# A2R-Lab/RBDReference

Hardware: AMD Instinct MI355X
Metric: batched RNEA+grad evals/s (7-DoF) (higher is better)
Workload: dtype f32

## Files before the change

rbdreference_amd/csrc/rbd_idsva_pipe.h:

```cpp
#pragma once
#include "rbd_idsva.h"

namespace rbdk {

constexpr bool ids_pipe_ok_() {
  if (!GRAD_IDSVA_OK) return false;
  if (n_groups() != 1 || grad_max_rows() != N) return false;
  if (N < 4) return false;
  if ((32 * GRAD_TILE) % 4 != 0 || GRAD_TILE % 2 != 0) return false;
  return true;
}
constexpr bool IDS_PIPE_OK = ids_pipe_ok_();

#define IDS_SB() __builtin_amdgcn_sched_barrier(0)
#ifndef IDS_FDG_LOAD_AT
#define IDS_FDG_LOAD_AT 0
#endif
#ifndef IDS_PIPE_LEAF_PARK
#define IDS_PIPE_LEAF_PARK 0
#endif
#ifndef IDS_PIPE_C_PARK
#define IDS_PIPE_C_PARK 0
#endif
#ifndef IDS_PIPE_PARK_UPTO
#define IDS_PIPE_PARK_UPTO 0
#endif
#ifndef IDS_PIPE_REG_ENTRIES_MAX
#define IDS_PIPE_REG_ENTRIES_MAX 50
#endif
constexpr int ids_pipe_rows_a(int rows) {
  for (int a = 0; a < rows; ++a)
    if (ids_regs_for(rows, a) <= IDS_PIPE_REG_ENTRIES_MAX && ids_tile_for(rows, a) <= IDS_TS) return a;
  return ids_rows_a(rows);
}
template <class X>
RBD_DEV void ids_undef(X& x) { asm volatile("" : "=v"(x)); }

template <class T, bool HAS_QDD, bool FDG = false>
__global__ __launch_bounds__(64, 2) void rnea_grad_idsva_pipe_kernel(const T* __restrict__ q, const T* __restrict__ qd,
                                                                    const T* __restrict__ qdd, T grav, int use_damping,
                                                                    long long B, T* __restrict__ c_out,
                                                                    T* __restrict__ dcdu, const T* __restrict__ minv_pk) {
  static_assert(sizeof(T) == 4, "fp32 kernel");
  extern __shared__ __attribute__((aligned(16))) unsigned char smem_raw[];
  T* tile = reinterpret_cast<T*>(smem_raw);
  const int lane = threadIdx.x;
  constexpr int CFGS = 64;
  constexpr int TS = IDS_TS;
  constexpr int row0 = 0, rows = N, last = N - 1;
  constexpr int ra = ids_pipe_rows_a(rows);
  static_assert(ids_tile_for(rows, ra) <= IDS_TS, "tile overflow");
  constexpr int rs = rows - ra;
  constexpr int PEND = ra * GRAD_ROW;
  constexpr int RW = GRAD_TILE;
  constexpr int VE = 4;
  constexpr int NV = 32 * RW / VE;
  constexpr int NRD = (NV + 63) / 64;
  constexpr int NVC = CFGS * N / VE;
  constexpr int NRC = (NVC + 63) / 64;
  typedef T V __attribute__((ext_vector_type(VE)));
  const long long ntiles = (B + CFGS - 1) / CFGS;
  long long t = blockIdx.x;
  if (t >= ntiles) return;
  T* my = tile + lane * TS;
  int gdim = (int)gridDim.x;
  asm volatile("" : "+s"(gdim));

  JTrig<T> tr[N];
  T qv[N], qdv[N], qddv[N];
  T qn[N], qdn[N], qddn[N];
  T Sv[N][6], Pd[N][6], Pdd[N][6];
  T cv[N];
  T Rm[3][3], pw[3], v[6], a[6];
  T E[RW];
  T mk[FDG ? FDC_NP : 1];
  long long tcur = 0;

  auto load_inputs = [&](long long tt, bool dummy) {
    const long long c0 = tt * CFGS;
    const long long rm = dummy ? 1 : B - c0;
    unsigned lo = (unsigned)((lane < rm ? lane : (int)rm - 1) * N);
    asm volatile("" : "+v"(lo));
    const T* qt = q + c0 * N + lo;
    const T* qdt = qd + c0 * N + lo;
    const T* qddt = HAS_QDD ? qdd + c0 * N + lo : nullptr;
    sfor<0, N>([&](auto J) {
      constexpr int j = decltype(J)::value;
      qn[j] = qt[j];
      qdn[j] = qdt[j];
      if constexpr (HAS_QDD) qddn[j] = qddt[j]; else qddn[j] = T(0);
    });
  };
  auto settle_inputs = [&]() {
    sfor<0, N>([&](auto J) {
      constexpr int j = decltype(J)::value;
      qn[j] = launder(qn[j]); qdn[j] = launder(qdn[j]); qddn[j] = launder(qddn[j]);
    });
  };
  auto take_inputs = [&]() {
    sfor<0, N>([&](auto J) { constexpr int j = decltype(J)::value; qv[j] = qn[j]; qdv[j] = qdn[j]; qddv[j] = qddn[j]; });
  };
  auto trig_chunk = [&](auto J0_, auto J1_) {
    constexpr int J0 = decltype(J0_)::value, J1 = decltype(J1_)::value;
    T mx = T(0);
    sfor<J0, J1>([&](auto J) { constexpr int j = decltype(J)::value; mx = __builtin_fmaxf(mx, __builtin_fabsf(qv[j])); });
    if (__builtin_expect(__builtin_amdgcn_ballot_w64(!(mx <= 8192.0f)) != 0, 0)) {
      sfor<J0, J1>([&](auto J) { constexpr int j = decltype(J)::value; sincos_wide_(qv[j], &tr[j].s, &tr[j].c); });
    } else {
      sfor<J0, J1>([&](auto J) { constexpr int j = decltype(J)::value; sincos_core_(qv[j], &tr[j].s, &tr[j].c); });
    }
  };

  auto fwd_body = [&](auto J) {
    constexpr int j = decltype(J)::value;
    constexpr int k = AXIS[j], ka = (k + 1) % 3, kb = (k + 2) % 3;
    constexpr bool root = PARENT[j] < 0;
    T Tm[3][3];
    sfor<0, 3>([&](auto R_) {
      sfor<0, 3>([&](auto C_) {
        constexpr int r = decltype(R_)::value, c = decltype(C_)::value;
        if constexpr (root) {
          Tm[r][c] = T(Et_(j, c, r));
        } else {
          T acc = T(0);
          sfor<0, 3>([&](auto M_) {
            constexpr int m = decltype(M_)::value;
            constexpr double e = Et_(j, c, m);
            if constexpr (e == 1.0) acc = acc + Rm[r][m];
            else if constexpr (e == -1.0) acc = acc - Rm[r][m];
            else if constexpr (e != 0.0) acc = fma_(T(e), Rm[r][m], acc);
          });
          Tm[r][c] = acc;
        }
      });
    });
    T pn[3];
    sfor<0, 3>([&](auto R_) {
      constexpr int r = decltype(R_)::value;
      if constexpr (root) {
        pn[r] = T(rt_(j, r));
      } else {
        T acc = pw[r];
        sfor<0, 3>([&](auto M_) {
          constexpr int m = decltype(M_)::value;
          constexpr double e = rt_(j, m);
          if constexpr (e != 0.0) acc = fma_(T(e), Rm[r][m], acc);
        });
        pn[r] = acc;
      }
    });
    sfor<0, 3>([&](auto R_) {
      constexpr int r = decltype(R_)::value;
      Rm[r][ka] = fma_(tr[j].c, Tm[r][ka], tr[j].s * Tm[r][kb]);
      Rm[r][kb] = fma_(tr[j].c, Tm[r][kb], -(tr[j].s * Tm[r][ka]));
      Rm[r][k] = Tm[r][k];
      pw[r] = pn[r];
    });
    const T ang[3] = {Rm[0][k], Rm[1][k], Rm[2][k]};
    T sl[3];
    cross3(pw, ang, sl);
    sfor<0, 3>([&](auto R_) { constexpr int r = decltype(R_)::value; Sv[j][r] = ang[r]; Sv[j][3 + r] = sl[r]; });
    if constexpr (root) {
      sfor<0, 6>([&](auto R_) { Pd[j][decltype(R_)::value] = T(0); });
      Pdd[j][0] = T(0); Pdd[j][1] = T(0); Pdd[j][2] = T(0);
      Pdd[j][3] = grav * ang[1];
      Pdd[j][4] = -(grav * ang[0]);
      Pdd[j][5] = T(0);
      sfor<0, 6>([&](auto R_) {
        constexpr int r = decltype(R_)::value;
        v[r] = Sv[j][r] * qdv[j];
        a[r] = Sv[j][r] * qddv[j];
      });
      a[5] -= grav;
    } else {
      T t1[6];
      crm6(v, Sv[j], Pd[j]);
      crm6(a, Sv[j], t1);
      crm6_add(v, Pd[j], t1, Pdd[j]);
      sfor<0, 6>([&](auto R_) {
        constexpr int r = decltype(R_)::value;
        v[r] = fma_(Sv[j][r], qdv[j], v[r]);
        a[r] = fma_(Sv[j][r], qddv[j], fma_(Pd[j][r], qdv[j], a[r]));
      });
    }
  };
  auto park = [&](auto J) {
    constexpr int j = decltype(J)::value;
    if constexpr (j > row0 && j < last && j <= IDS_PIPE_PARK_UPTO) {
      my[ids_park_slot(row0, rows, ra, j, 0)] = tr[j].s; my[ids_park_slot(row0, rows, ra, j, 1)] = tr[j].c;
      my[ids_park_slot(row0, rows, ra, j, 2)] = qdv[j]; my[ids_park_slot(row0, rows, ra, j, 3)] = qddv[j];
    }
    if constexpr (j == last && (IDS_PIPE_LEAF_PARK && ids_leaf_parks(row0, rows, ra))) {
      my[ids_leaf_slot(row0, rows, ra, 0)] = tr[j].s; my[ids_leaf_slot(row0, rows, ra, 1)] = tr[j].c;
      my[ids_leaf_slot(row0, rows, ra, 2)] = qdv[j]; my[ids_leaf_slot(row0, rows, ra, 3)] = qddv[j];
    }
  };

  auto backward = [&](long long tnext_or_t, bool dummy) {
    RInertia<T> IC;
    SymB<T> SC;
    T pmC[6], fC[6];
    sfor_down<row0, row0 + rows>([&](auto J) {
      constexpr int j = decltype(J)::value;
      constexpr int k = AXIS[j], ka = (k + 1) % 3, kb = (k + 2) % 3;
      constexpr bool top = j >= rs;
      if constexpr (j == rs && ra > 1 && (IDS_PIPE_C_PARK && ids_c_parks(row0, rows, ra))) {
        asm volatile("" ::: "memory");
        sfor<rs + 1, row0 + rows>([&](auto JC) { constexpr int jc = decltype(JC)::value; cv[jc] = my[ids_c_slot(row0, rows, ra, jc - rs - 1)]; });
      }
      if constexpr (j > row0 && j < last && j <= IDS_PIPE_PARK_UPTO) {
        asm volatile("" ::: "memory");
        tr[j].s = my[ids_park_slot(row0, rows, ra, j, 0)]; tr[j].c = my[ids_park_slot(row0, rows, ra, j, 1)];
        qdv[j] = my[ids_park_slot(row0, rows, ra, j, 2)]; qddv[j] = my[ids_park_slot(row0, rows, ra, j, 3)];
#ifndef RBD_EXP_NO_PIN_READBACK
        IDS_SB();
#endif
      }
      if constexpr (FDG && j == row0 + (rows > IDS_FDG_LOAD_AT ? IDS_FDG_LOAD_AT : rows - 1)) {
        IDS_SB();
        int lo = lane;
        asm volatile("" : "+v"(lo));
        const T* mp = minv_pk + (size_t)tcur * (FDC_NP * 64) + lo;
#ifdef RBD_FDG_EXP_NOLOAD
        sfor<0, FDC_NP>([&](auto S_) { constexpr int s_ = decltype(S_)::value; mk[s_] = launder(T(1) + T(s_)); });
#else
        sfor<0, FDC_NP>([&](auto S_) { constexpr int s_ = decltype(S_)::value; mk[s_] = mp[s_ * 64]; });
#endif
        IDS_SB();
      }
      RInertia<T> L;
      T cw[3];
      sfor<0, 3>([&](auto R_) {
        constexpr int r = decltype(R_)::value;
        T acc = pw[r];
        sfor<0, 3>([&](auto M_) {
          constexpr int m = decltype(M_)::value;
          constexpr double e = com_(j, m);
          if constexpr (e != 0.0) acc = fma_(T(e), Rm[r][m], acc);
        });
        cw[r] = acc;
      });
      L.m = T(mass_(j));
      sfor<0, 3>([&](auto R_) { L.h[decltype(R_)::value] = T(mass_(j)) * cw[decltype(R_)::value]; });
      {
        T A[3][3];
        sfor<0, 3>([&](auto R_) {
          sfor<0, 3>([&](auto C_) {
            constexpr int r = decltype(R_)::value, c = decltype(C_)::value;
            T acc = T(0);
            sfor<0, 3>([&](auto M_) {
              constexpr int m = decltype(M_)::value;
              constexpr double e = Ic_(j, m, c);
              if constexpr (e != 0.0) acc = fma_(T(e), Rm[r][m], acc);
            });
            A[r][c] = acc;
          });
        });
        const T cc = fma_(cw[0], cw[0], fma_(cw[1], cw[1], cw[2] * cw[2]));
        constexpr int IR[6] = {0, 0, 0, 1, 1, 2}, IC_[6] = {0, 1, 2, 1, 2, 2};
        sfor<0, 6>([&](auto E_) {
          constexpr int e = decltype(E_)::value, r = IR[e], c = IC_[e];
          T s = fma_(A[r][0], Rm[c][0], fma_(A[r][1], Rm[c][1], A[r][2] * Rm[c][2]));
          s = fma_(-L.h[r], cw[c], s);
          if constexpr (r == c) s = fma_(L.m, cc, s);
          L.I[e] = s;
        });
      }
      T pm[6];
      rin_apply(L, v, pm);
      if constexpr (j == last) {
        T Ia[6];
        rin_apply(L, a, Ia);
        fxv_add(v, pm, Ia, fC);
        IC = L;
        sfor<0, 6>([&](auto R_) { constexpr int r = decltype(R_)::value; pmC[r] = pm[r]; });
      } else {
        T t[6];
        rin_apply_acc(L, a, fC, t);
        fxv_add(v, pm, t, fC);
        IC.m += L.m;
        sfor<0, 3>([&](auto R_) { constexpr int r = decltype(R_)::value; IC.h[r] += L.h[r]; });
        sfor<0, 6>([&](auto R_) { constexpr int r = decltype(R_)::value; IC.I[r] += L.I[r]; pmC[r] += pm[r]; });
      }
      {
        const T w[3] = {v[0], v[1], v[2]}, u[3] = {v[3], v[4], v[5]};
        const T Ifull[3][3] = {{L.I[0], L.I[1], L.I[2]}, {L.I[1], L.I[3], L.I[4]}, {L.I[2], L.I[4], L.I[5]}};
        const T uh = fma_(u[0], L.h[0], fma_(u[1], L.h[1], u[2] * L.h[2]));
        constexpr int IR[6] = {0, 0, 0, 1, 1, 2}, IC_[6] = {0, 1, 2, 1, 2, 2};
        sfor<0, 6>([&](auto E_) {
          constexpr int e = decltype(E_)::value, r = IR[e], c = IC_[e];
          constexpr int r1 = (r + 1) % 3, r2 = (r + 2) % 3, c1 = (c + 1) % 3, c2 = (c + 2) % 3;
          const T base = (j == last) ? T(0) : SC.TL[e];
          if constexpr (r == c) {
            const T d = fma_(-L.h[r], u[r], fma_(w[r1], Ifull[r2][r], fma_(-w[r2], Ifull[r1][r], uh)));
            SC.TL[e] = fma_(T(2), d, base);
          } else {
            T x = fma_(w[r1], Ifull[r2][c], fma_(-w[r2], Ifull[r1][c], base));
            x = fma_(w[c1], Ifull[c2][r], fma_(-w[c2], Ifull[c1][r], x));
            SC.TL[e] = fma_(-L.h[r], u[c], fma_(-u[r], L.h[c], x));
          }
        });
        sfor<0, 3>([&](auto R_) {
          constexpr int r = decltype(R_)::value, r1 = (r + 1) % 3, r2 = (r + 2) % 3;
          const T base = (j == last) ? T(0) : SC.G[r];
          SC.G[r] = fma_(L.m, u[r], fma_(w[r1], L.h[r2], fma_(-w[r2], L.h[r1], base)));
        });
      }
      cv[j] = dot6(Sv[j], fC);
      if constexpr (j > rs && (IDS_PIPE_C_PARK && ids_c_parks(row0, rows, ra))) my[ids_c_slot(row0, rows, ra, j - rs - 1)] = cv[j];
      T t1[6], t2[6], t3[6], t4[6];
      {
        T y3[6], s1[6], yf[6];
        rin_apply(IC, Sv[j], t1);
        sym_apply(SC, Sv[j], s1);
        fxv_sub(Sv[j], pmC, s1, t4);
        rin_apply(IC, Pdd[j], y3);
        fxv_add(Sv[j], fC, y3, yf);
        if constexpr (PARENT[j] < 0) {
          sfor<0, 6>([&](auto R_) {
            constexpr int r = decltype(R_)::value;
            t3[r] = yf[r];
            t2[r] = fma_(T(2), s1[r], -t4[r]);
          });
        } else {
          T y2[6], ys[6];
          rin_apply(IC, Pd[j], y2);
          sym_apply_acc(SC, Pd[j], yf, ys);
          fxv_add(Pd[j], pmC, ys, t3);
          sfor<0, 6>([&](auto R_) {
            constexpr int r = decltype(R_)::value;
            t2[r] = fma_(T(2), y2[r] + s1[r], -t4[r]);
          });
        }
      }
      sfor<row0, j + 1>([&](auto JJ) {
        constexpr int jj = decltype(JJ)::value;
        T dq_ij, dqd_ij;
        if constexpr (PARENT[jj] < 0) {
          dq_ij = fma_(t1[3], Pdd[jj][3], t1[4] * Pdd[jj][4]);
          dqd_ij = dot6(t4, Sv[jj]);
        } else {
          dq_ij = dot6_acc(t1, Pdd[jj], dot6(t4, Pd[jj]));
          dqd_ij = fma_(T(2), dot6(t1, Pd[jj]), dot6(t4, Sv[jj]));
        }
        if constexpr (jj == j) dqd_ij += sel(use_damping != 0, T(DAMPING[j]), T(0));
        if constexpr (top) {
          my[(j - rs) * GRAD_ROW + jj] = dq_ij;
          my[(j - rs) * GRAD_ROW + N + jj] = dqd_ij;
        } else {
          E[(j - row0) * GRAD_ROW + jj] = dq_ij;
          E[(j - row0) * GRAD_ROW + N + jj] = dqd_ij;
        }
        if constexpr (jj != j) {
          const T e3 = dot6(Sv[jj], t3), e2 = dot6(Sv[jj], t2);
          if constexpr (!top) {
            E[(jj - row0) * GRAD_ROW + j] = e3;
            E[(jj - row0) * GRAD_ROW + N + j] = e2;
          } else if constexpr (jj < rs) {
            constexpr int slot = PEND + ((jj - row0) * ra + (j - rs)) * 2;
            my[slot] = e3;
            my[slot + 1] = e2;
          } else {
            my[(jj - rs) * GRAD_ROW + j] = e3;
            my[(jj - rs) * GRAD_ROW + N + j] = e2;
          }
        }
      });
      if constexpr (j == row0 + (rows > IDS_PREFETCH_AT ? IDS_PREFETCH_AT : rows - 1)) {
        IDS_SB();
        load_inputs(tnext_or_t, dummy);
        IDS_SB();
      }
      if constexpr (j == last && (IDS_PIPE_LEAF_PARK && ids_leaf_parks(row0, rows, ra))) {
        asm volatile("" ::: "memory");
        tr[j].s = my[ids_leaf_slot(row0, rows, ra, 0)]; tr[j].c = my[ids_leaf_slot(row0, rows, ra, 1)];
        qdv[j] = my[ids_leaf_slot(row0, rows, ra, 2)]; qddv[j] = my[ids_leaf_slot(row0, rows, ra, 3)];
      }
      if constexpr (j > row0) {
        sfor<0, 6>([&](auto R_) {
          constexpr int r = decltype(R_)::value;
          v[r] = fma_(-Sv[j][r], qdv[j], v[r]);
          a[r] = fma_(-Sv[j][r], qddv[j], fma_(-Pd[j][r], qdv[j], a[r]));
        });
        T Tm[3][3];
        sfor<0, 3>([&](auto R_) {
          constexpr int r = decltype(R_)::value;
          Tm[r][ka] = fma_(tr[j].c, Rm[r][ka], -(tr[j].s * Rm[r][kb]));
          Tm[r][kb] = fma_(tr[j].s, Rm[r][ka], tr[j].c * Rm[r][kb]);
          Tm[r][k] = Rm[r][k];
        });
        sfor<0, 3>([&](auto R_) {
          sfor<0, 3>([&](auto C_) {
            constexpr int r = decltype(R_)::value, c = decltype(C_)::value;
            T acc = T(0);
            sfor<0, 3>([&](auto M_) {
              constexpr int m = decltype(M_)::value;
              constexpr double e = Et_(j, m, c);
              if constexpr (e == 1.0) acc = acc + Tm[r][m];
              else if constexpr (e == -1.0) acc = acc - Tm[r][m];
              else if constexpr (e != 0.0) acc = fma_(T(e), Tm[r][m], acc);
            });
            Rm[r][c] = acc;
          });
        });
        sfor<0, 3>([&](auto R_) {
          constexpr int r = decltype(R_)::value;
          T acc = pw[r];
          sfor<0, 3>([&](auto M_) {
            constexpr int m = decltype(M_)::value;
            constexpr double e = rt_(j, m);
            if constexpr (e != 0.0) acc = fma_(T(-e), Rm[r][m], acc);
          });
          pw[r] = acc;
        });
      }
    });
  };

  auto readback = [&]() {
    sfor<rs, row0 + rows>([&](auto R_) {
      sfor<0, GRAD_ROW>([&](auto C_) {
        constexpr int r = decltype(R_)::value, c = decltype(C_)::value;
        E[(r - row0) * GRAD_ROW + c] = my[(r - rs) * GRAD_ROW + c];
      });
    });
    sfor<row0, rs>([&](auto JJ) {
      sfor<rs, row0 + rows>([&](auto JA) {
        constexpr int jj = decltype(JJ)::value, ja = decltype(JA)::value;
        constexpr int slot = PEND + ((jj - row0) * ra + (ja - rs)) * 2;
        E[(jj - row0) * GRAD_ROW + ja] = my[slot];
        E[(jj - row0) * GRAD_ROW + N + ja] = my[slot + 1];
      });
    });
  };
  auto image_write = [&](int ln, int h) {
    if ((ln >> 5) == h) {
      T* img = tile + (ln & 31) * RW;
      typedef T V2 __attribute__((ext_vector_type(2)));
      sfor<0, RW / 2>([&](auto K_) {
        constexpr int k = decltype(K_)::value;
        V2 x; x[0] = E[2 * k]; x[1] = E[2 * k + 1];
        reinterpret_cast<V2*>(img)[k] = x;
      });
    }
  };
  auto image_read = [&](int ln, V (&buf)[NRD]) {
    const V* src = reinterpret_cast<const V*>(tile);
    sfor<0, NRD>([&](auto I_) {
      constexpr int i = decltype(I_)::value;
      if constexpr ((i + 1) * 64 <= NV) buf[i] = src[ln + 64 * i];
      else buf[i] = src[(ln + 64 * i < NV) ? ln + 64 * i : 0];
    });
  };
  auto image_store = [&](int ln, long long cfg0, int h, const V (&buf)[NRD]) {
    V* dst = reinterpret_cast<V*>(dcdu + (cfg0 + 32 * h) * GRAD_TILE);
    sfor<0, NRD>([&](auto I_) {
      constexpr int i = decltype(I_)::value;
      if constexpr ((i + 1) * 64 <= NV) dst[ln + 64 * i] = buf[i];
      else { if (ln + 64 * i < NV) dst[ln + 64 * i] = buf[i]; }
    });
  };
  auto flush_half_plain = [&](int ln, long long cfg0, int nvalid, int h) {
    image_write(ln, h);
    IDS_WAVE_SYNC();
    const int nv = nvalid - 32 * h;
    if (nv >= 32) {
      V buf[NRD];
      image_read(ln, buf);
      image_store(ln, cfg0, h, buf);
    } else if (nv > 0) {
      T* gdst = dcdu + (cfg0 + 32 * h) * GRAD_TILE;
#pragma unroll 2
      for (int g = ln; g < nv * RW; g += 64) gdst[g] = tile[g];
    }
    IDS_WAVE_SYNC();
  };
  auto flush_c_plain = [&](int ln, long long cfg0, int nvalid) {
    if (c_out != nullptr) {
      sfor<0, N>([&](auto J) { constexpr int j = decltype(J)::value; tile[ln * N + j] = cv[j]; });
      IDS_WAVE_SYNC();
      T* cdst = c_out + cfg0 * N;
      if (nvalid == CFGS && (CFGS * N) % VE == 0) {
        sfor<0, NRC>([&](auto I_) {
          constexpr int i = decltype(I_)::value;
          if (ln + 64 * i < NVC) reinterpret_cast<V*>(cdst)[ln + 64 * i] = reinterpret_cast<const V*>(tile)[ln + 64 * i];
        });
      } else {
        for (int g = ln; g < nvalid * N; g += 64) cdst[g] = tile[g];
      }
      IDS_WAVE_SYNC();
    }
  };

  load_inputs(t, false);
  settle_inputs();
  bool first = true;
  long long pcfg0 = 0;
  constexpr bool c_flat = (CFGS * N) % VE == 0;
  for (;;) {
    V buf[NRD], cbuf[NRC];
    sfor<0, NRD>([&](auto I_) { ids_undef(buf[decltype(I_)::value]); });
    sfor<0, NRC>([&](auto I_) { ids_undef(cbuf[decltype(I_)::value]); });
    const long long cfg0 = t * CFGS;
    const long long tnext = t + gdim;
    const bool has_next = tnext < ntiles;
    int ln = lane;
    asm volatile("" : "+v"(ln));

    take_inputs();
    IDS_SB();
    constexpr int TA = N >= 6 ? 2 : 1, TB = N >= 6 ? 4 : 2;
    trig_chunk(std::integral_constant<int, 0>{}, std::integral_constant<int, TA>{});
    IDS_SB();
    __builtin_amdgcn_s_waitcnt(0xC07F);
    if (!first) {
      image_write(ln, 0);
      IDS_WAVE_SYNC();
      image_read(ln, buf);
    }
    IDS_SB();
    trig_chunk(std::integral_constant<int, TA>{}, std::integral_constant<int, TB>{});
    IDS_SB();
    if (!first) {
      image_store(ln, pcfg0, 0, buf);
      IDS_WAVE_SYNC();
      image_write(ln, 1);
      IDS_WAVE_SYNC();
      image_read(ln, buf);
    }
    IDS_SB();
    trig_chunk(std::integral_constant<int, TB>{}, std::integral_constant<int, N>{});
    fwd_body(std::integral_constant<int, 0>{});
    IDS_SB();
    if (!first) {
      image_store(ln, pcfg0, 1, buf);
      IDS_WAVE_SYNC();
      if (c_out != nullptr) {
        sfor<0, N>([&](auto J) { constexpr int j = decltype(J)::value; tile[ln * N + j] = cv[j]; });
        IDS_WAVE_SYNC();
        if constexpr (c_flat) {
          sfor<0, NRC>([&](auto I_) {
            constexpr int i = decltype(I_)::value;
            cbuf[i] = reinterpret_cast<const V*>(tile)[(ln + 64 * i < NVC) ? ln + 64 * i : 0];
          });
        }
      }
    }
    IDS_SB();
    fwd_body(std::integral_constant<int, 1>{});
    IDS_SB();
    if (!first && c_out != nullptr) {
      T* cdst = c_out + pcfg0 * N;
      if constexpr (c_flat) {
        sfor<0, NRC>([&](auto I_) {
          constexpr int i = decltype(I_)::value;
          if (ln + 64 * i < NVC) reinterpret_cast<V*>(cdst)[ln + 64 * i] = cbuf[i];
        });
      } else {
        for (int g = ln; g < CFGS * N; g += 64) cdst[g] = tile[g];
      }
    }
    IDS_WAVE_SYNC();
    park(std::integral_constant<int, 1>{});
    sfor<2, N>([&](auto J) { fwd_body(J); park(J); });

    tcur = t;
    backward(has_next ? tnext : t, !has_next);

    readback();
#ifdef RBD_FDG_EXP_NOPROD
    if constexpr (FDG) { sfor<0, FDC_NP>([&](auto S_) { constexpr int s_ = decltype(S_)::value; E[s_] += mk[s_]; }); }
    if constexpr (false) {
#else
    if constexpr (FDG) {
#endif
      sfor<0, GRAD_ROW>([&](auto C_) {
        constexpr int c = decltype(C_)::value;
        T x[N];
        sfor<0, N>([&](auto K_) { constexpr int k = decltype(K_)::value; x[k] = E[k * GRAD_ROW + c]; });
        sfor<0, N>([&](auto I_) {
          constexpr int i = decltype(I_)::value;
          T o = -(mk[fdc_sym(i, 0)] * x[0]);
          sfor<1, N>([&](auto K_) { constexpr int k = decltype(K_)::value; o = fma_(-mk[fdc_sym(i, k)], x[k], o); });
          E[i * GRAD_ROW + c] = o;
        });
      });
    }
    settle_inputs();
    IDS_WAVE_SYNC();
    if (!has_next) break;
    first = false;
    pcfg0 = cfg0;
    t = tnext;
  }
  {
    const long long cfg0 = t * CFGS;
    const long long rem = B - cfg0;
    const int nvalid = rem < CFGS ? (int)rem : CFGS;
    int ln = lane;
    asm volatile("" : "+v"(ln));
    flush_half_plain(ln, cfg0, nvalid, 0);
    flush_half_plain(ln, cfg0, nvalid, 1);
    flush_c_plain(ln, cfg0, nvalid);
  }
}

}
```

rbdreference_amd/csrc/rbd_world.h:

```cpp
#pragma once
#include "rbd_spatial.h"

namespace rbdk {

template <class T>
RBD_DEV void cross3(const T (&a)[3], const T (&b)[3], T (&o)[3]) {
  o[0] = fma_(a[1], b[2], -(a[2] * b[1]));
  o[1] = fma_(a[2], b[0], -(a[0] * b[2]));
  o[2] = fma_(a[0], b[1], -(a[1] * b[0]));
}
template <class T>
RBD_DEV void cross3_acc(const T (&a)[3], const T (&b)[3], T (&o)[3]) {
  o[0] = fma_(a[1], b[2], fma_(-a[2], b[1], o[0]));
  o[1] = fma_(a[2], b[0], fma_(-a[0], b[2], o[1]));
  o[2] = fma_(a[0], b[1], fma_(-a[1], b[0], o[2]));
}
template <class T>
RBD_DEV void crm6(const T (&v)[6], const T (&x)[6], T (&o)[6]) {
  const T w[3] = {v[0], v[1], v[2]}, u[3] = {v[3], v[4], v[5]};
  const T xa[3] = {x[0], x[1], x[2]}, xb[3] = {x[3], x[4], x[5]};
  T oa[3], ob[3];
  cross3(w, xa, oa);
  cross3(u, xa, ob);
  cross3_acc(w, xb, ob);
  o[0] = oa[0]; o[1] = oa[1]; o[2] = oa[2]; o[3] = ob[0]; o[4] = ob[1]; o[5] = ob[2];
}
template <class T>
struct RInertia {
  T m, h[3], I[6];
};
template <class T>
RBD_DEV void rin_apply(const RInertia<T>& R, const T (&x)[6], T (&y)[6]) {
  const T w[3] = {x[0], x[1], x[2]}, u[3] = {x[3], x[4], x[5]};
  T top[3] = {fma_(R.I[0], w[0], fma_(R.I[1], w[1], R.I[2] * w[2])),
              fma_(R.I[1], w[0], fma_(R.I[3], w[1], R.I[4] * w[2])),
              fma_(R.I[2], w[0], fma_(R.I[4], w[1], R.I[5] * w[2]))};
  cross3_acc(R.h, u, top);
  T hw[3];
  cross3(R.h, w, hw);
  y[0] = top[0]; y[1] = top[1]; y[2] = top[2];
  y[3] = fma_(R.m, u[0], -hw[0]); y[4] = fma_(R.m, u[1], -hw[1]); y[5] = fma_(R.m, u[2], -hw[2]);
}
template <class T>
struct SymB {
  T TL[6], G[3];
};
template <class T>
RBD_DEV void sym_apply(const SymB<T>& S, const T (&x)[6], T (&y)[6]) {
  const T a[3] = {x[0], x[1], x[2]}, b[3] = {x[3], x[4], x[5]};
  T top[3] = {fma_(S.TL[0], a[0], fma_(S.TL[1], a[1], S.TL[2] * a[2])),
              fma_(S.TL[1], a[0], fma_(S.TL[3], a[1], S.TL[4] * a[2])),
              fma_(S.TL[2], a[0], fma_(S.TL[4], a[1], S.TL[5] * a[2]))};
  cross3_acc(S.G, b, top);
  T ga[3];
  cross3(S.G, a, ga);
  y[0] = top[0]; y[1] = top[1]; y[2] = top[2];
  y[3] = -ga[0]; y[4] = -ga[1]; y[5] = -ga[2];
}

template <class T>
RBD_DEV T dot6_acc(const T (&x)[6], const T (&y)[6], T acc) {
  return fma_(x[5], y[5], fma_(x[4], y[4], fma_(x[3], y[3], fma_(x[2], y[2], fma_(x[1], y[1], fma_(x[0], y[0], acc))))));
}
template <class T>
RBD_DEV void fxv_add(const T (&v)[6], const T (&b)[6], const T (&acc)[6], T (&r)[6]) {
  const T r0 = fma_(v[1], b[2], fma_(-v[2], b[1], fma_(v[4], b[5], fma_(-v[5], b[4], acc[0]))));
  const T r1 = fma_(v[2], b[0], fma_(-v[0], b[2], fma_(v[5], b[3], fma_(-v[3], b[5], acc[1]))));
  const T r2 = fma_(v[0], b[1], fma_(-v[1], b[0], fma_(v[3], b[4], fma_(-v[4], b[3], acc[2]))));
  const T r3 = fma_(v[1], b[5], fma_(-v[2], b[4], acc[3]));
  const T r4 = fma_(v[2], b[3], fma_(-v[0], b[5], acc[4]));
  const T r5 = fma_(v[0], b[4], fma_(-v[1], b[3], acc[5]));
  r[0] = r0; r[1] = r1; r[2] = r2; r[3] = r3; r[4] = r4; r[5] = r5;
}
template <class T>
RBD_DEV void fxv_sub(const T (&v)[6], const T (&b)[6], const T (&acc)[6], T (&r)[6]) {
  const T r0 = fma_(-v[1], b[2], fma_(v[2], b[1], fma_(-v[4], b[5], fma_(v[5], b[4], acc[0]))));
  const T r1 = fma_(-v[2], b[0], fma_(v[0], b[2], fma_(-v[5], b[3], fma_(v[3], b[5], acc[1]))));
  const T r2 = fma_(-v[0], b[1], fma_(v[1], b[0], fma_(-v[3], b[4], fma_(v[4], b[3], acc[2]))));
  const T r3 = fma_(-v[1], b[5], fma_(v[2], b[4], acc[3]));
  const T r4 = fma_(-v[2], b[3], fma_(v[0], b[5], acc[4]));
  const T r5 = fma_(-v[0], b[4], fma_(v[1], b[3], acc[5]));
  r[0] = r0; r[1] = r1; r[2] = r2; r[3] = r3; r[4] = r4; r[5] = r5;
}
template <class T>
RBD_DEV void crm6_add(const T (&v)[6], const T (&x)[6], const T (&acc)[6], T (&o)[6]) {
  const T w[3] = {v[0], v[1], v[2]}, u[3] = {v[3], v[4], v[5]};
  const T xa[3] = {x[0], x[1], x[2]}, xb[3] = {x[3], x[4], x[5]};
  T oa[3] = {acc[0], acc[1], acc[2]}, ob[3] = {acc[3], acc[4], acc[5]};
  cross3_acc(w, xa, oa);
  cross3_acc(u, xa, ob);
  cross3_acc(w, xb, ob);
  o[0] = oa[0]; o[1] = oa[1]; o[2] = oa[2]; o[3] = ob[0]; o[4] = ob[1]; o[5] = ob[2];
}
template <class T>
RBD_DEV void rin_apply_acc(const RInertia<T>& R, const T (&x)[6], const T (&acc)[6], T (&y)[6]) {
  const T w[3] = {x[0], x[1], x[2]}, u[3] = {x[3], x[4], x[5]};
  T top[3] = {fma_(R.I[0], w[0], fma_(R.I[1], w[1], fma_(R.I[2], w[2], acc[0]))),
              fma_(R.I[1], w[0], fma_(R.I[3], w[1], fma_(R.I[4], w[2], acc[1]))),
              fma_(R.I[2], w[0], fma_(R.I[4], w[1], fma_(R.I[5], w[2], acc[2])))};
  cross3_acc(R.h, u, top);
  y[0] = top[0]; y[1] = top[1]; y[2] = top[2];
  T bot[3] = {fma_(R.m, u[0], acc[3]), fma_(R.m, u[1], acc[4]), fma_(R.m, u[2], acc[5])};
  cross3_acc(w, R.h, bot);
  y[3] = bot[0]; y[4] = bot[1]; y[5] = bot[2];
}
template <class T>
RBD_DEV void sym_apply_acc(const SymB<T>& S, const T (&x)[6], const T (&acc)[6], T (&y)[6]) {
  const T a[3] = {x[0], x[1], x[2]}, b[3] = {x[3], x[4], x[5]};
  T top[3] = {fma_(S.TL[0], a[0], fma_(S.TL[1], a[1], fma_(S.TL[2], a[2], acc[0]))),
              fma_(S.TL[1], a[0], fma_(S.TL[3], a[1], fma_(S.TL[4], a[2], acc[1]))),
              fma_(S.TL[2], a[0], fma_(S.TL[4], a[1], fma_(S.TL[5], a[2], acc[2])))};
  cross3_acc(S.G, b, top);
  T bot[3] = {acc[3], acc[4], acc[5]};
  cross3_acc(a, S.G, bot);
  y[0] = top[0]; y[1] = top[1]; y[2] = top[2]; y[3] = bot[0]; y[4] = bot[1]; y[5] = bot[2];
}

struct TreePlan {
  int sub[N > 0 ? N : 1] = {};
  int heavy[N > 0 ? N : 1] = {};
  int head[N > 0 ? N : 1] = {};
  int pos[N > 0 ? N : 1] = {};
  int leaf[N > 0 ? N : 1] = {};
  int len[N > 0 ? N : 1] = {};
  int park[N > 0 ? N : 1] = {};
  int cross0[N > 0 ? N : 1] = {};
  int rootidx[N > 0 ? N : 1] = {};
  int side_head[N > 0 ? N : 1] = {};
  bool on_side[N > 0 ? N : 1] = {};
  bool any_side = false;
  int wave_of[N > 0 ? N : 1] = {};
  int wave_len[16] = {};
  int inch_off[17] = {};
  int n_waves = 0;
  int n_cross = 0, n_park = 0, max_len = 0, n_roots = 0;
  constexpr TreePlan() {
    for (int i = 0; i < N; ++i) rootidx[i] = PARENT[i] < 0 ? n_roots++ : rootidx[PARENT[i]];
    for (int i = 0; i < N; ++i) sub[i] = 1;
    for (int i = N - 1; i >= 0; --i)
      if (PARENT[i] >= 0) sub[PARENT[i]] += sub[i];
    for (int i = 0; i < N; ++i) heavy[i] = -1;
    for (int i = 0; i < N; ++i) {
      const int p = PARENT[i];
      if (p >= 0 && (heavy[p] < 0 || sub[i] > sub[heavy[p]])) heavy[p] = i;
    }
    for (int i = 0; i < N; ++i) {
      const int p = PARENT[i];
      if (p >= 0 && heavy[p] == i) { head[i] = head[p]; pos[i] = pos[p] + 1; }
      else { head[i] = i; pos[i] = 0; }
    }
    for (int i = 0; i < N; ++i) { leaf[i] = i; len[i] = 0; }
    for (int i = 0; i < N; ++i) {
      const int h = head[i];
      if (pos[i] + 1 > len[h]) { len[h] = pos[i] + 1; leaf[h] = i; }
    }
    for (int i = 0; i < N; ++i) {
      if (head[i] == i) {
        if (len[i] > max_len) max_len = len[i];
        if (PARENT[i] >= 0) park[i] = n_park++;
      }
    }
    for (int j = 0; j < N; ++j) {
      cross0[j] = n_cross;
      for (int x = PARENT[j]; x >= 0; x = PARENT[x])
        if (head[x] != head[j]) ++n_cross;
    }
    for (int r = 0; r < N; ++r) side_head[r] = -1;
    for (int h = 0; h < N; ++h) {
      const int p = PARENT[h];
      if (head[h] != h || p < 0) continue;
      int rt = h;
      while (PARENT[rt] >= 0) rt = PARENT[rt];
      if (head[p] != rt) continue;
      if (sub[h] < 4) continue;
      const int ri = rootidx[h];
      if (side_head[ri] < 0 || sub[h] > sub[side_head[ri]]) side_head[ri] = h;
    }
    for (int j = 0; j < N; ++j) {
      const int sh = side_head[rootidx[j]];
      bool in = false;
      if (sh >= 0)
        for (int x = j; x >= 0; x = PARENT[x])
          if (x == sh) in = true;
      on_side[j] = in;
      any_side = any_side || in;
    }
    {
      int base[N > 0 ? N : 1] = {};
      int w = 0;
      for (int r = 0; r < N; ++r)
        if (PARENT[r] < 0) { base[rootidx[r]] = w; w += 1 + (side_head[rootidx[r]] >= 0 ? 1 : 0); }
      n_waves = w;
      for (int j = 0; j < N; ++j) wave_of[j] = base[rootidx[j]] + (on_side[j] ? 1 : 0);
      if (w <= 16) {
        int load[16] = {};
        for (int hd = 0; hd < N; ++hd)
          if (head[hd] == hd) load[wave_of[hd]] += DEPTH[leaf[hd]] + 1 + 2 * len[hd];
        for (int x = 0; x < N; ++x) {
          const int p = PARENT[x];
          if (head[x] != x || p < 0) continue;
          const int sh = side_head[rootidx[x]];
          if (sh < 0 || on_side[x]) continue;
          int rt = x;
          while (PARENT[rt] >= 0) rt = PARENT[rt];
          if (head[p] != rt) continue;
          bool above = false;
          for (int y = PARENT[sh]; y >= 0; y = PARENT[y]) above = above || y == p;
          if (!above) continue;
          int cost = 0;
          for (int hd = 0; hd < N; ++hd) {
            bool in = false;
            for (int y = hd; y >= 0; y = PARENT[y]) in = in || y == x;
            if (in && head[hd] == hd) cost += DEPTH[leaf[hd]] + 1 + 2 * len[hd];
          }
          const int wm = wave_of[rt];
          int best = -1;
          for (int k = 0; k < w; ++k)
            if (k != wm && (best < 0 || load[k] < load[best])) best = k;
          if (best < 0 || load[best] + cost >= load[wm]) continue;
          for (int j = 0; j < N; ++j) {
            bool in = false;
            for (int y = j; y >= 0; y = PARENT[y]) in = in || y == x;
            if (in) wave_of[j] = best;
          }
          load[best] += cost;
          load[wm] -= cost;
        }
      }
      for (int j = 0; j < N; ++j)
        if (head[j] == j && wave_of[j] < 16 && len[j] > wave_len[wave_of[j]]) wave_len[wave_of[j]] = len[j];
      for (int k = 0; k < 16; ++k) inch_off[k + 1] = inch_off[k] + wave_len[k] * (wave_len[k] - 1);
    }
  }
};
constexpr TreePlan TP{};
constexpr bool is_chain_head(int i) { return TP.head[i] == i; }
constexpr int chain_head_of(int i) { return TP.head[i]; }
constexpr int chain_leaf(int h) { return TP.leaf[h]; }
constexpr bool in_chain(int j, int h) { return TP.head[j] == h; }
constexpr int pos_in_chain(int j) { return TP.pos[j]; }
constexpr int max_chain_len() { return TP.max_len; }
constexpr int cross_rank(int jj, int j) {
  int k = TP.cross0[j];
  for (int x = PARENT[j]; x >= 0 && x != jj; x = PARENT[x])
    if (TP.head[x] != TP.head[j]) ++k;
  return k;
}
constexpr int n_cross_pairs() { return TP.n_cross; }
constexpr int park_rank(int h) { return TP.park[h]; }
constexpr int n_parked_chains() { return TP.n_park; }
constexpr int tree_n_roots() { return TP.n_roots; }

template <class T>
struct WState {
  T R[3][3], p[3], v[6], a[6];
};

template <int J, class T>
RBD_DEV void ws_down(WState<T>& s, const JTrig<T>& g, T qd, T qdd, T grav, T (&Sv)[6], T (&Pd)[6], T (&Pdd)[6]) {
  constexpr int k = AXIS[J], ka = (k + 1) % 3, kb = (k + 2) % 3;
  constexpr bool root = PARENT[J] < 0;
  T Tm[3][3];
  sfor<0, 3>([&](auto R_) {
    sfor<0, 3>([&](auto C_) {
      constexpr int r = decltype(R_)::value, c = decltype(C_)::value;
      if constexpr (root) {
        Tm[r][c] = T(Et_(J, c, r));
      } else {
        T acc = T(0);
        sfor<0, 3>([&](auto M_) {
          constexpr int m = decltype(M_)::value;
          constexpr double e = Et_(J, c, m);
          if constexpr (e == 1.0) acc = acc + s.R[r][m];
          else if constexpr (e == -1.0) acc = acc - s.R[r][m];
          else if constexpr (e != 0.0) acc = fma_(T(e), s.R[r][m], acc);
        });
        Tm[r][c] = acc;
      }
    });
  });
  T pn[3];
  sfor<0, 3>([&](auto R_) {
    constexpr int r = decltype(R_)::value;
    if constexpr (root) {
      pn[r] = T(rt_(J, r));
    } else {
      T acc = s.p[r];
      sfor<0, 3>([&](auto M_) {
        constexpr int m = decltype(M_)::value;
        constexpr double e = rt_(J, m);
        if constexpr (e != 0.0) acc = fma_(T(e), s.R[r][m], acc);
      });
      pn[r] = acc;
    }
  });
  if constexpr (JTYPE[J] == 0) {
    sfor<0, 3>([&](auto R_) {
      constexpr int r = decltype(R_)::value;
      s.R[r][ka] = fma_(g.c, Tm[r][ka], g.s * Tm[r][kb]);
      s.R[r][kb] = fma_(g.c, Tm[r][kb], -(g.s * Tm[r][ka]));
      s.R[r][k] = Tm[r][k];
      s.p[r] = pn[r];
    });
    const T ang[3] = {s.R[0][k], s.R[1][k], s.R[2][k]};
    T sl[3];
    cross3(s.p, ang, sl);
    sfor<0, 3>([&](auto R_) { constexpr int r = decltype(R_)::value; Sv[r] = ang[r]; Sv[3 + r] = sl[r]; });
  } else {
    sfor<0, 3>([&](auto R_) {
      constexpr int r = decltype(R_)::value;
      sfor<0, 3>([&](auto C_) { constexpr int c = decltype(C_)::value; s.R[r][c] = Tm[r][c]; });
      s.p[r] = fma_(g.s, Tm[r][k], pn[r]);
      Sv[r] = T(0);
      Sv[3 + r] = Tm[r][k];
    });
  }
  if constexpr (root) {
    sfor<0, 6>([&](auto R_) { Pd[decltype(R_)::value] = T(0); });
    Pdd[0] = T(0); Pdd[1] = T(0); Pdd[2] = T(0);
    Pdd[3] = JTYPE[J] == 0 ? grav * Sv[1] : T(0);
    Pdd[4] = JTYPE[J] == 0 ? -(grav * Sv[0]) : T(0);
    Pdd[5] = T(0);
    sfor<0, 6>([&](auto R_) {
      constexpr int r = decltype(R_)::value;
      s.v[r] = Sv[r] * qd;
      s.a[r] = Sv[r] * qdd;
    });
    s.a[5] -= grav;
  } else {
    T t1[6];
    crm6(s.v, Sv, Pd);
    crm6(s.a, Sv, t1);
    crm6_add(s.v, Pd, t1, Pdd);
    sfor<0, 6>([&](auto R_) {
      constexpr int r = decltype(R_)::value;
      s.v[r] = fma_(Sv[r], qd, s.v[r]);
      s.a[r] = fma_(Sv[r], qdd, fma_(Pd[r], qd, s.a[r]));
    });
  }
}

template <int J, class T>
RBD_DEV void ws_up(WState<T>& s, const JTrig<T>& g, T qd, T qdd, const T (&Sv)[6], const T (&Pd)[6]) {
  constexpr int k = AXIS[J], ka = (k + 1) % 3, kb = (k + 2) % 3;
  sfor<0, 6>([&](auto R_) {
    constexpr int r = decltype(R_)::value;
    s.v[r] = fma_(-Sv[r], qd, s.v[r]);
    s.a[r] = fma_(-Sv[r], qdd, fma_(-Pd[r], qd, s.a[r]));
  });
  T Tm[3][3];
  sfor<0, 3>([&](auto R_) {
    constexpr int r = decltype(R_)::value;
    Tm[r][ka] = fma_(g.c, s.R[r][ka], -(g.s * s.R[r][kb]));
    Tm[r][kb] = fma_(g.s, s.R[r][ka], g.c * s.R[r][kb]);
    Tm[r][k] = s.R[r][k];
  });
  sfor<0, 3>([&](auto R_) {
    sfor<0, 3>([&](auto C_) {
      constexpr int r = decltype(R_)::value, c = decltype(C_)::value;
      T acc = T(0);
      sfor<0, 3>([&](auto M_) {
        constexpr int m = decltype(M_)::value;
        constexpr double e = Et_(J, m, c);
        if constexpr (e == 1.0) acc = acc + Tm[r][m];
        else if constexpr (e == -1.0) acc = acc - Tm[r][m];
        else if constexpr (e != 0.0) acc = fma_(T(e), Tm[r][m], acc);
      });
      s.R[r][c] = acc;
    });
  });
  sfor<0, 3>([&](auto R_) {
    constexpr int r = decltype(R_)::value;
    T acc = s.p[r];
    sfor<0, 3>([&](auto M_) {
      constexpr int m = decltype(M_)::value;
      constexpr double e = rt_(J, m);
      if constexpr (e != 0.0) acc = fma_(T(-e), s.R[r][m], acc);
    });
    s.p[r] = acc;
  });
}

constexpr int TREE_COMP_SCALARS = 31;
template <class T>
struct Comp {
  RInertia<T> IC;
  SymB<T> SC;
  T pm[6], f[6];
};
template <class T>
RBD_DEV void comp_add(Comp<T>& a, const Comp<T>& b) {
  a.IC.m += b.IC.m;
  sfor<0, 3>([&](auto R_) { constexpr int r = decltype(R_)::value; a.IC.h[r] += b.IC.h[r]; a.SC.G[r] += b.SC.G[r]; });
  sfor<0, 6>([&](auto R_) {
    constexpr int r = decltype(R_)::value;
    a.IC.I[r] += b.IC.I[r]; a.SC.TL[r] += b.SC.TL[r]; a.pm[r] += b.pm[r]; a.f[r] += b.f[r];
  });
}
template <int J, class T>
RBD_DEV void comp_local(const WState<T>& s, Comp<T>& L) {
  T cw[3];
  sfor<0, 3>([&](auto R_) {
    constexpr int r = decltype(R_)::value;
    T acc = s.p[r];
    sfor<0, 3>([&](auto M_) {
      constexpr int m = decltype(M_)::value;
      constexpr double e = com_(J, m);
      if constexpr (e != 0.0) acc = fma_(T(e), s.R[r][m], acc);
    });
    cw[r] = acc;
  });
  L.IC.m = T(mass_(J));
  sfor<0, 3>([&](auto R_) { L.IC.h[decltype(R_)::value] = T(mass_(J)) * cw[decltype(R_)::value]; });
  {
    T A[3][3];
    sfor<0, 3>([&](auto R_) {
      sfor<0, 3>([&](auto C_) {
        constexpr int r = decltype(R_)::value, c = decltype(C_)::value;
        T acc = T(0);
        sfor<0, 3>([&](auto M_) {
          constexpr int m = decltype(M_)::value;
          constexpr double e = Ic_(J, m, c);
          if constexpr (e != 0.0) acc = fma_(T(e), s.R[r][m], acc);
        });
        A[r][c] = acc;
      });
    });
    const T cc = fma_(cw[0], cw[0], fma_(cw[1], cw[1], cw[2] * cw[2]));
    constexpr int IR[6] = {0, 0, 0, 1, 1, 2}, IC_[6] = {0, 1, 2, 1, 2, 2};
    sfor<0, 6>([&](auto E_) {
      constexpr int e = decltype(E_)::value, r = IR[e], c = IC_[e];
      T x = fma_(A[r][0], s.R[c][0], fma_(A[r][1], s.R[c][1], A[r][2] * s.R[c][2]));
      const T mcc = L.IC.h[r] * cw[c];
      if constexpr (r == c) x += fma_(L.IC.m, cc, -mcc); else x -= mcc;
      L.IC.I[e] = x;
    });
  }
  T Ia[6];
  rin_apply(L.IC, s.v, L.pm);
  rin_apply(L.IC, s.a, Ia);
  fxv_add(s.v, L.pm, Ia, L.f);
  {
    const T w[3] = {s.v[0], s.v[1], s.v[2]}, u[3] = {s.v[3], s.v[4], s.v[5]};
    const T Ifull[3][3] = {{L.IC.I[0], L.IC.I[1], L.IC.I[2]}, {L.IC.I[1], L.IC.I[3], L.IC.I[4]}, {L.IC.I[2], L.IC.I[4], L.IC.I[5]}};
    T K[3][3];
    sfor<0, 3>([&](auto C_) {
      constexpr int c = decltype(C_)::value;
      const T col[3] = {Ifull[0][c], Ifull[1][c], Ifull[2][c]};
      T o[3];
      cross3(w, col, o);
      K[0][c] = o[0]; K[1][c] = o[1]; K[2][c] = o[2];
    });
    const T uh2 = T(2) * fma_(u[0], L.IC.h[0], fma_(u[1], L.IC.h[1], u[2] * L.IC.h[2]));
    constexpr int IR[6] = {0, 0, 0, 1, 1, 2}, IC_[6] = {0, 1, 2, 1, 2, 2};
    sfor<0, 6>([&](auto E_) {
      constexpr int e = decltype(E_)::value, r = IR[e], c = IC_[e];
      T x = K[r][c] + K[c][r];
      x = fma_(-L.IC.h[r], u[c], fma_(-u[r], L.IC.h[c], x));
      if constexpr (r == c) x += uh2;
      L.SC.TL[e] = x;
    });
    T g[3];
    cross3(w, L.IC.h, g);
    sfor<0, 3>([&](auto R_) { constexpr int r = decltype(R_)::value; L.SC.G[r] = fma_(L.IC.m, u[r], g[r]); });
  }
}
template <bool ROOT, class T>
RBD_DEV void tvectors(const Comp<T>& C, const T (&Sj)[6], const T (&Pdj)[6], const T (&Pddj)[6], T (&t1)[6], T (&t2)[6], T (&t3)[6], T (&t4)[6]) {
  T y3[6], s1[6], yf[6];
  rin_apply(C.IC, Sj, t1);
  sym_apply(C.SC, Sj, s1);
  fxv_sub(Sj, C.pm, s1, t4);
  rin_apply(C.IC, Pddj, y3);
  fxv_add(Sj, C.f, y3, yf);
  if constexpr (ROOT) {
    sfor<0, 6>([&](auto R_) {
      constexpr int r = decltype(R_)::value;
      t3[r] = yf[r];
      t2[r] = fma_(T(2), s1[r], -t4[r]);
    });
  } else {
    T y2[6], ys[6];
    rin_apply(C.IC, Pdj, y2);
    sym_apply_acc(C.SC, Pdj, yf, ys);
    fxv_add(Pdj, C.pm, ys, t3);
    sfor<0, 6>([&](auto R_) {
      constexpr int r = decltype(R_)::value;
      t2[r] = fma_(T(2), y2[r] + s1[r], -t4[r]);
    });
  }
}
template <class T, class F>
RBD_DEV void comp_each(Comp<T>& c, F&& f) {
  f(std::integral_constant<int, 0>{}, c.IC.m);
  sfor<0, 3>([&](auto R_) { constexpr int r = decltype(R_)::value; f(std::integral_constant<int, 1 + r>{}, c.IC.h[r]); });
  sfor<0, 6>([&](auto R_) { constexpr int r = decltype(R_)::value; f(std::integral_constant<int, 4 + r>{}, c.IC.I[r]); });
  sfor<0, 6>([&](auto R_) { constexpr int r = decltype(R_)::value; f(std::integral_constant<int, 10 + r>{}, c.SC.TL[r]); });
  sfor<0, 3>([&](auto R_) { constexpr int r = decltype(R_)::value; f(std::integral_constant<int, 16 + r>{}, c.SC.G[r]); });
  sfor<0, 6>([&](auto R_) { constexpr int r = decltype(R_)::value; f(std::integral_constant<int, 19 + r>{}, c.pm[r]); });
  sfor<0, 6>([&](auto R_) { constexpr int r = decltype(R_)::value; f(std::integral_constant<int, 25 + r>{}, c.f[r]); });
}

template <int CPI, int SST, class V>
RBD_DEV void flush_image_rows_buf(const V* src, __amdgpu_buffer_rsrc_t rs, int voff, int soff, int dstride_bytes, int fsub, int fe) {
  static_assert(sizeof(V) == 16, "16-byte vectors");
  typedef unsigned U4 __attribute__((ext_vector_type(4)));
  constexpr int IT = (64 + CPI - 1) / CPI;
  constexpr int BATCH = 16 < IT ? 16 : IT;
  sfor<0, (IT + BATCH - 1) / BATCH>([&](auto G_) {
    constexpr int g = decltype(G_)::value;
    V buf[BATCH];
    sfor<0, BATCH>([&](auto I_) {
      constexpr int i = decltype(I_)::value, it = g * BATCH + i;
      if constexpr (it < IT) {
        const int cfg = it * CPI + fsub;
        if constexpr ((it + 1) * CPI <= 64) buf[i] = src[cfg * SST + fe];
        else buf[i] = src[(cfg < 64 ? cfg : 63) * SST + fe];
      }
    });
    sfor<0, BATCH>([&](auto I_) {
      constexpr int i = decltype(I_)::value, it = g * BATCH + i;
      if constexpr (it < IT) {
        if constexpr ((it + 1) * CPI <= 64) {
          __builtin_amdgcn_raw_buffer_store_b128(__builtin_bit_cast(U4, buf[i]), rs, voff, soff + it * CPI * dstride_bytes, 0);
        } else {
          if (it * CPI + fsub < 64) __builtin_amdgcn_raw_buffer_store_b128(__builtin_bit_cast(U4, buf[i]), rs, voff, soff + it * CPI * dstride_bytes, 0);
        }
      }
    });
  });
}

template <int CPI, int SST, bool BATCHED = true, class V>
RBD_DEV void flush_image_rows(const V* src, V* dst, long long dstride, int fsub, int fe, int nvalid) {
  constexpr int IT = (64 + CPI - 1) / CPI;
  constexpr int BATCH = (int)(256 / sizeof(V)) < IT ? (int)(256 / sizeof(V)) : IT;
  if (BATCHED && nvalid == 64) {
    sfor<0, (IT + BATCH - 1) / BATCH>([&](auto G_) {
      constexpr int g = decltype(G_)::value;
      V buf[BATCH];
      sfor<0, BATCH>([&](auto I_) {
        constexpr int i = decltype(I_)::value, it = g * BATCH + i;
        if constexpr (it < IT) {
          const int cfg = it * CPI + fsub;
          if constexpr ((it + 1) * CPI <= 64) buf[i] = src[cfg * SST + fe];
          else buf[i] = src[(cfg < 64 ? cfg : 63) * SST + fe];
        }
      });
      sfor<0, BATCH>([&](auto I_) {
        constexpr int i = decltype(I_)::value, it = g * BATCH + i;
        if constexpr (it < IT) {
          const int cfg = it * CPI + fsub;
          if constexpr ((it + 1) * CPI <= 64) dst[cfg * dstride + fe] = buf[i];
          else if (cfg < 64) dst[cfg * dstride + fe] = buf[i];
        }
      });
    });
  } else {
#pragma unroll 4
    for (int c0 = 0; c0 < 64; c0 += CPI) {
      const int cfg = c0 + fsub;
      if (cfg < nvalid) dst[cfg * dstride + fe] = src[cfg * SST + fe];
    }
  }
}

}
```

Baseline: 8.246 billion.

## Trim scalar/address overhead in IDSVA pipe kernel and fold negation in rin_apply

Switches tile indices to 32-bit unsigned, precomputes the last tile's row count, and builds load/store addresses from byte offsets and SGPR bases with immediate offsets. The trig range check is hoisted into a single ballot per tile that is reused across chunks, and the first-iteration flag becomes an SGPR value. Bounds checks on tile over-reads are replaced by static asserts, and rin_apply gains a negated cross product so the sign flips fold into the FMAs. An optional b32 image-write path is added but left off by default. The aim is fewer VALU/SALU instructions and registers, at the cost of relying on over-reads staying inside the tile and on 32-bit tile counts.

```diff
diff --git a/rbdreference_amd/csrc/rbd_idsva_pipe.h b/rbdreference_amd/csrc/rbd_idsva_pipe.h
--- a/rbdreference_amd/csrc/rbd_idsva_pipe.h
+++ b/rbdreference_amd/csrc/rbd_idsva_pipe.h
@@ -25,6 +25,9 @@
 #ifndef IDS_PIPE_PARK_UPTO
 #define IDS_PIPE_PARK_UPTO 0
 #endif
+#ifndef IDS_PIPE_IMG_B32
+#define IDS_PIPE_IMG_B32 0
+#endif
 #ifndef IDS_PIPE_REG_ENTRIES_MAX
 #define IDS_PIPE_REG_ENTRIES_MAX 50
 #endif
@@ -33,6 +36,7 @@
     if (ids_regs_for(rows, a) <= IDS_PIPE_REG_ENTRIES_MAX && ids_tile_for(rows, a) <= IDS_TS) return a;
   return ids_rows_a(rows);
 }
+RBD_DEV bool ids_sflag(int x) { asm volatile("" : "+s"(x)); return x != 0; }
 template <class X>
 RBD_DEV void ids_undef(X& x) { asm volatile("" : "=v"(x)); }
 
@@ -59,8 +63,10 @@
   constexpr int NVC = CFGS * N / VE;
   constexpr int NRC = (NVC + 63) / 64;
   typedef T V __attribute__((ext_vector_type(VE)));
-  const long long ntiles = (B + CFGS - 1) / CFGS;
-  long long t = blockIdx.x;
+  constexpr bool IMG_OVER_OK = NRD * 64 * VE <= 64 * TS, CIMG_OVER_OK = NRC * 64 * VE <= 64 * TS;
+  const unsigned ntiles = (unsigned)((B + CFGS - 1) / CFGS);
+  const int lastrows = (int)(B - (long long)(ntiles - 1) * CFGS);
+  unsigned t = blockIdx.x;
   if (t >= ntiles) return;
   T* my = tile + lane * TS;
   int gdim = (int)gridDim.x;
@@ -74,16 +80,17 @@
   T Rm[3][3], pw[3], v[6], a[6];
   T E[RW];
   T mk[FDG ? FDC_NP : 1];
-  long long tcur = 0;
-
-  auto load_inputs = [&](long long tt, bool dummy) {
-    const long long c0 = tt * CFGS;
-    const long long rm = dummy ? 1 : B - c0;
-    unsigned lo = (unsigned)((lane < rm ? lane : (int)rm - 1) * N);
+  unsigned tcur = 0;
+
+  auto load_inputs = [&](unsigned tt, bool dummy) {
+    const long long c0 = (long long)tt * CFGS;
+    const int rm = dummy ? 1 : (tt + 1 == ntiles ? lastrows : CFGS);
+    unsigned lo = (unsigned)(lane < rm ? lane : rm - 1) * (unsigned)(N * sizeof(T));
     asm volatile("" : "+v"(lo));
-    const T* qt = q + c0 * N + lo;
-    const T* qdt = qd + c0 * N + lo;
-    const T* qddt = HAS_QDD ? qdd + c0 * N + lo : nullptr;
+    auto at = [&](const T* base) { return reinterpret_cast<const T*>(reinterpret_cast<const char*>(base + c0 * N) + lo); };
+    const T* qt = at(q);
+    const T* qdt = at(qd);
+    const T* qddt = HAS_QDD ? at(qdd) : nullptr;
     sfor<0, N>([&](auto J) {
       constexpr int j = decltype(J)::value;
       qn[j] = qt[j];
@@ -100,11 +107,17 @@
   auto take_inputs = [&]() {
     sfor<0, N>([&](auto J) { constexpr int j = decltype(J)::value; qv[j] = qn[j]; qdv[j] = qdn[j]; qddv[j] = qddn[j]; });
   };
-  auto trig_chunk = [&](auto J0_, auto J1_) {
+  auto trig_range = [&]() -> int {
+    T mx = T(0);
+    sfor<0, N>([&](auto J) { constexpr int j = decltype(J)::value; mx = __builtin_fmaxf(mx, __builtin_fabsf(qv[j])); });
+    const unsigned long long b = __builtin_amdgcn_ballot_w64(!(mx <= 8192.0f));
+    int w = (int)((unsigned)b | (unsigned)(b >> 32));
+    asm volatile("" : "+s"(w));
+    return w;
+  };
+  auto trig_chunk = [&](int wide, auto J0_, auto J1_) {
     constexpr int J0 = decltype(J0_)::value, J1 = decltype(J1_)::value;
-    T mx = T(0);
-    sfor<J0, J1>([&](auto J) { constexpr int j = decltype(J)::value; mx = __builtin_fmaxf(mx, __builtin_fabsf(qv[j])); });
-    if (__builtin_expect(__builtin_amdgcn_ballot_w64(!(mx <= 8192.0f)) != 0, 0)) {
+    if (__builtin_expect(ids_sflag(wide), 0)) {
       sfor<J0, J1>([&](auto J) { constexpr int j = decltype(J)::value; sincos_wide_(qv[j], &tr[j].s, &tr[j].c); });
     } else {
       sfor<J0, J1>([&](auto J) { constexpr int j = decltype(J)::value; sincos_core_(qv[j], &tr[j].s, &tr[j].c); });
@@ -196,7 +209,7 @@
     }
   };
 
-  auto backward = [&](long long tnext_or_t, bool dummy) {
+  auto backward = [&](unsigned tnext_or_t, bool dummy) {
     RInertia<T> IC;
     SymB<T> SC;
     T pmC[6], fC[6];
@@ -436,28 +449,43 @@
   auto image_write = [&](int ln, int h) {
     if ((ln >> 5) == h) {
       T* img = tile + (ln & 31) * RW;
+#if IDS_PIPE_IMG_B32
+      typedef __attribute__((address_space(3))) T LT;
+      LT* im = (LT*)img;
+      asm volatile("" : "+v"(im));
+      sfor<0, RW>([&](auto K_) { constexpr int k = decltype(K_)::value; im[k] = E[k]; });
+#else
       typedef T V2 __attribute__((ext_vector_type(2)));
       sfor<0, RW / 2>([&](auto K_) {
         constexpr int k = decltype(K_)::value;
         V2 x; x[0] = E[2 * k]; x[1] = E[2 * k + 1];
         reinterpret_cast<V2*>(img)[k] = x;
       });
+#endif
     }
   };
   auto image_read = [&](int ln, V (&buf)[NRD]) {
     const V* src = reinterpret_cast<const V*>(tile);
     sfor<0, NRD>([&](auto I_) {
       constexpr int i = decltype(I_)::value;
-      if constexpr ((i + 1) * 64 <= NV) buf[i] = src[ln + 64 * i];
-      else buf[i] = src[(ln + 64 * i < NV) ? ln + 64 * i : 0];
+      static_assert((i + 1) * 64 <= NV || IMG_OVER_OK, "the over-read leaves the tile");
+      buf[i] = src[ln + 64 * i];
     });
   };
   auto image_store = [&](int ln, long long cfg0, int h, const V (&buf)[NRD]) {
-    V* dst = reinterpret_cast<V*>(dcdu + (cfg0 + 32 * h) * GRAD_TILE);
+    char* dst = reinterpret_cast<char*>(dcdu + (cfg0 + 32 * h) * GRAD_TILE);
+    const unsigned lo = (unsigned)ln * (unsigned)sizeof(V);
+    constexpr unsigned IMM = 4096, NG = (NRD * 64 * sizeof(V) + IMM - 1) / IMM;
+    typedef __attribute__((address_space(1))) char GC;
+    typedef __attribute__((address_space(1))) V GV;
+    GC* dg[NG];
+    sfor<0, NG>([&](auto G_) { constexpr int g = decltype(G_)::value; dg[g] = (GC*)(dst + g * IMM); asm volatile("" : "+s"(dg[g])); });
     sfor<0, NRD>([&](auto I_) {
       constexpr int i = decltype(I_)::value;
-      if constexpr ((i + 1) * 64 <= NV) dst[ln + 64 * i] = buf[i];
-      else { if (ln + 64 * i < NV) dst[ln + 64 * i] = buf[i]; }
+      constexpr unsigned off = 64 * i * sizeof(V);
+      GV* p = (GV*)(dg[off / IMM] + lo + off % IMM);
+      if constexpr ((i + 1) * 64 <= NV) *p = buf[i];
+      else { if (ln + 64 * i < NV) *p = buf[i]; }
     });
   };
   auto flush_half_plain = [&](int ln, long long cfg0, int nvalid, int h) {
@@ -494,34 +522,36 @@
 
   load_inputs(t, false);
   settle_inputs();
-  bool first = true;
+  int prev = 0;
   long long pcfg0 = 0;
   constexpr bool c_flat = (CFGS * N) % VE == 0;
   for (;;) {
     V buf[NRD], cbuf[NRC];
     sfor<0, NRD>([&](auto I_) { ids_undef(buf[decltype(I_)::value]); });
     sfor<0, NRC>([&](auto I_) { ids_undef(cbuf[decltype(I_)::value]); });
-    const long long cfg0 = t * CFGS;
-    const long long tnext = t + gdim;
+    const long long cfg0 = (long long)t * CFGS;
+    const unsigned tnext = t + (unsigned)gdim;
     const bool has_next = tnext < ntiles;
     int ln = lane;
     asm volatile("" : "+v"(ln));
+    asm volatile("" : "+s"(prev));
 
     take_inputs();
+    const int wide = trig_range();
     IDS_SB();
     constexpr int TA = N >= 6 ? 2 : 1, TB = N >= 6 ? 4 : 2;
-    trig_chunk(std::integral_constant<int, 0>{}, std::integral_constant<int, TA>{});
+    trig_chunk(wide, std::integral_constant<int, 0>{}, std::integral_constant<int, TA>{});
     IDS_SB();
     __builtin_amdgcn_s_waitcnt(0xC07F);
-    if (!first) {
+    if (ids_sflag(prev)) {
       image_write(ln, 0);
       IDS_WAVE_SYNC();
       image_read(ln, buf);
     }
     IDS_SB();
-    trig_chunk(std::integral_constant<int, TA>{}, std::integral_constant<int, TB>{});
-    IDS_SB();
-    if (!first) {
+    trig_chunk(wide, std::integral_constant<int, TA>{}, std::integral_constant<int, TB>{});
+    IDS_SB();
+    if (ids_sflag(prev)) {
       image_store(ln, pcfg0, 0, buf);
       IDS_WAVE_SYNC();
       image_write(ln, 1);
@@ -529,10 +559,10 @@
       image_read(ln, buf);
     }
     IDS_SB();
-    trig_chunk(std::integral_constant<int, TB>{}, std::integral_constant<int, N>{});
+    trig_chunk(wide, std::integral_constant<int, TB>{}, std::integral_constant<int, N>{});
     fwd_body(std::integral_constant<int, 0>{});
     IDS_SB();
-    if (!first) {
+    if (ids_sflag(prev)) {
       image_store(ln, pcfg0, 1, buf);
       IDS_WAVE_SYNC();
       if (c_out != nullptr) {
@@ -541,7 +571,8 @@
         if constexpr (c_flat) {
           sfor<0, NRC>([&](auto I_) {
             constexpr int i = decltype(I_)::value;
-            cbuf[i] = reinterpret_cast<const V*>(tile)[(ln + 64 * i < NVC) ? ln + 64 * i : 0];
+            static_assert(CIMG_OVER_OK, "the over-read leaves the tile");
+            cbuf[i] = reinterpret_cast<const V*>(tile)[ln + 64 * i];
           });
         }
       }
@@ -549,12 +580,15 @@
     IDS_SB();
     fwd_body(std::integral_constant<int, 1>{});
     IDS_SB();
-    if (!first && c_out != nullptr) {
+    if (ids_sflag(prev) && c_out != nullptr) {
       T* cdst = c_out + pcfg0 * N;
       if constexpr (c_flat) {
+        const unsigned lo = (unsigned)ln * (unsigned)sizeof(V);
         sfor<0, NRC>([&](auto I_) {
           constexpr int i = decltype(I_)::value;
-          if (ln + 64 * i < NVC) reinterpret_cast<V*>(cdst)[ln + 64 * i] = cbuf[i];
+          V* p = reinterpret_cast<V*>(reinterpret_cast<char*>(cdst) + lo + 64 * i * sizeof(V));
+          if constexpr ((i + 1) * 64 <= NVC) *p = cbuf[i];
+          else { if (ln + 64 * i < NVC) *p = cbuf[i]; }
         });
       } else {
         for (int g = ln; g < CFGS * N; g += 64) cdst[g] = tile[g];
@@ -589,12 +623,12 @@
     settle_inputs();
     IDS_WAVE_SYNC();
     if (!has_next) break;
-    first = false;
+    prev = 1;
     pcfg0 = cfg0;
     t = tnext;
   }
   {
-    const long long cfg0 = t * CFGS;
+    const long long cfg0 = (long long)t * CFGS;
     const long long rem = B - cfg0;
     const int nvalid = rem < CFGS ? (int)rem : CFGS;
     int ln = lane;
diff --git a/rbdreference_amd/csrc/rbd_world.h b/rbdreference_amd/csrc/rbd_world.h
--- a/rbdreference_amd/csrc/rbd_world.h
+++ b/rbdreference_amd/csrc/rbd_world.h
@@ -8,6 +8,12 @@
   o[0] = fma_(a[1], b[2], -(a[2] * b[1]));
   o[1] = fma_(a[2], b[0], -(a[0] * b[2]));
   o[2] = fma_(a[0], b[1], -(a[1] * b[0]));
+}
+template <class T>
+RBD_DEV void cross3_neg(const T (&a)[3], const T (&b)[3], T (&o)[3]) {
+  o[0] = fma_(-a[1], b[2], a[2] * b[1]);
+  o[1] = fma_(-a[2], b[0], a[0] * b[2]);
+  o[2] = fma_(-a[0], b[1], a[1] * b[0]);
 }
 template <class T>
 RBD_DEV void cross3_acc(const T (&a)[3], const T (&b)[3], T (&o)[3]) {
@@ -36,10 +42,10 @@
               fma_(R.I[1], w[0], fma_(R.I[3], w[1], R.I[4] * w[2])),
               fma_(R.I[2], w[0], fma_(R.I[4], w[1], R.I[5] * w[2]))};
   cross3_acc(R.h, u, top);
-  T hw[3];
-  cross3(R.h, w, hw);
+  T nhw[3];
+  cross3_neg(R.h, w, nhw);
   y[0] = top[0]; y[1] = top[1]; y[2] = top[2];
-  y[3] = fma_(R.m, u[0], -hw[0]); y[4] = fma_(R.m, u[1], -hw[1]); y[5] = fma_(R.m, u[2], -hw[2]);
+  y[3] = fma_(R.m, u[0], nhw[0]); y[4] = fma_(R.m, u[1], nhw[1]); y[5] = fma_(R.m, u[2], nhw[2]);
 }
 template <class T>
 struct SymB {
```

After: 8.310 billion, median of 6. No clear change (+0.8%).
